# radiocosmology/cora

Hardware: AMD Instinct MI355X
Metric: sky-maps/sec (nside=1024, lmax=2048, 256 freq) (higher is better)
Workload: dtype f64

## Files before the change

cora_amd/csrc/common.h:

```cpp
#pragma once
#include <hip/hip_runtime.h>

#include <cstdarg>
#include <cstdint>
#include <cstdio>
#include <map>
#include <string>
#include <type_traits>
#include <vector>

#include "../../include/corahip.h"

void corahip_set_error(const char *fmt, ...);

struct corahip_prof_entry {
    double total_ms = 0.0;
    int launches = 0;
};

struct corahip_pending_event {
    std::string name;
    hipEvent_t e0, e1;
};

struct corahip_linefft_plan {
    int n = 0, P = 0, logP = 0, blu = 0;
    int Pct = 0;
    double2 *filt_ct = nullptr;
    double2 *tw = nullptr;
    double2 *chirp = nullptr;
    double2 *filt = nullptr;
    double2 *rtw = nullptr;
};

#define CORAHIP_NSCRATCH 12
struct corahip_ctx {
    int device = 0;
    hipStream_t stream = nullptr;
    hipStream_t stream2 = nullptr;
    hipEvent_t ev_fork = nullptr, ev_join = nullptr;
    int *k5_tickets = nullptr;
    unsigned *draw_slot_tab = nullptr;
    int draw_slot_lmax = -1;
    bool mt_plist_ready = false;
    hipStream_t gen_stream = nullptr;
    hipEvent_t ev_ring[8] = {};
    const void *draw_pending = nullptr;
    hipEvent_t t0 = nullptr, t1 = nullptr;
    bool profile = false;
    std::map<std::string, corahip_prof_entry> prof;
    std::vector<corahip_pending_event> pending;
    int num_cu = 256;
    size_t total_mem = 0;
    void *scratch[CORAHIP_NSCRATCH] = {};
    size_t scratch_bytes[CORAHIP_NSCRATCH] = {};
    const void *tt_pin[3] = {nullptr, nullptr, nullptr};
    uint64_t tt_pin_gen = 0;
    bool tt_pinned = false, tt_valid = false;
    hipStream_t tt_stream = nullptr;
    long pairs_key[4] = {-1, -1, -1, -1};
    void *pairs_ptr = nullptr;
    std::map<int, corahip_linefft_plan> linefft;
};

int corahip_ctx_scratch(corahip_ctx *ctx, int slot, size_t bytes, void **out);

struct StageTimer {
    corahip_ctx *ctx;
    hipEvent_t e0 = nullptr, e1 = nullptr;
    const char *name;
    hipStream_t stream;
    StageTimer(corahip_ctx *c, const char *n, hipStream_t on = nullptr, bool other = false) : ctx(c), name(n), stream(other ? on : c->stream) {
        if (ctx->profile) {
            (void)hipEventCreate(&e0);
            (void)hipEventCreate(&e1);
            (void)hipEventRecord(e0, stream);
        }
    }
    ~StageTimer() {
        if (ctx->profile) {
            (void)hipEventRecord(e1, stream);
            ctx->pending.push_back({name, e0, e1});
        }
    }
};

#define HIP_TRY(expr)                                                                       \
    do {                                                                                    \
        hipError_t _e = (expr);                                                             \
        if (_e != hipSuccess) {                                                             \
            corahip_set_error("%s failed: %s (%s:%d)", #expr, hipGetErrorString(_e),        \
                              __FILE__, __LINE__);                                          \
            return (int)_e;                                                                 \
        }                                                                                   \
    } while (0)

#define ARG_CHECK(cond)                                                                     \
    do {                                                                                    \
        if (!(cond)) {                                                                      \
            corahip_set_error("invalid argument: %s (%s:%d)", #cond, __FILE__, __LINE__);   \
            return CORAHIP_EINVAL;                                                          \
        }                                                                                   \
    } while (0)

#define LAUNCH_CHECK() HIP_TRY(hipGetLastError())


static inline unsigned grid_blocks(const corahip_ctx *ctx, long n, int per_cu = 16) {
    long blocks = (n + 255) / 256;
    const long cap = (long)ctx->num_cu * per_cu;
    if (blocks > cap) blocks = cap;
    return (unsigned)(blocks < 1 ? 1 : blocks);
}

static inline void partials_split(long count, int round, int *nb, long *per) {
    long b = (count + 8191) / 8192;
    if (b > 4096) b = 4096;
    long pr = (count + b - 1) / b;
    pr = (pr + round - 1) & ~(long)(round - 1);
    *nb = (int)((count + pr - 1) / pr);
    *per = pr;
}

static inline bool overlaps(const void *a, size_t na, const void *b, size_t nb) {
    const uintptr_t pa = (uintptr_t)a, pb = (uintptr_t)b;
    return a && b && pa < pb + nb && pb < pa + na;
}

static inline int log2_exact(int v) {
    int k = 0;
    while ((1 << k) < v) k++;
    return (1 << k) == v ? k : -1;
}

static inline bool is_aligned(const void *p, unsigned bytes) { return ((uintptr_t)p & (bytes - 1)) == 0; }

__host__ __device__ static inline long nalm_of(int lmax) { return (long)(lmax + 1) * (lmax + 2) / 2; }
__host__ __device__ static inline long alm_idx(int l, int m, int lmax) {
    return (long)m * (2 * lmax + 1 - m) / 2 + l;
}

__device__ static inline long alm_l_of_idx(long idx, int lmax) {
    const double b = 2.0 * lmax + 3.0;
    long m = (long)((b - sqrt(b * b - 8.0 * (double)idx)) * 0.5);
    m = m < 0 ? 0 : (m > lmax ? lmax : m);
    while (m > 0 && m * (2L * lmax + 3 - m) / 2 > idx) m--;
    while (m < lmax && (m + 1) * (2L * lmax + 2 - m) / 2 <= idx) m++;
    return idx - m * (2L * lmax + 1 - m) / 2;
}

typedef double d4_t __attribute__((ext_vector_type(4)));

template <int N, int J = 0, class Fn>
__device__ static inline void static_for(Fn &&f) {
    if constexpr (J < N) {
        f(std::integral_constant<int, J>{});
        static_for<N, J + 1>(f);
    }
}

__device__ static inline void block_sum2(double &a, double &b, double *red) {
#pragma unroll
    for (int o = 32; o >= 1; o >>= 1) {
        a += __shfl_down(a, o, 64);
        b += __shfl_down(b, o, 64);
    }
    const int lane = threadIdx.x & 63, wave = threadIdx.x >> 6;
    if (lane == 0) red[2 * wave] = a, red[2 * wave + 1] = b;
    __syncthreads();
    a = ((red[0] + red[2]) + red[4]) + red[6];
    b = ((red[1] + red[3]) + red[5]) + red[7];
}
```

cora_amd/csrc/ctx.hip:

```cpp
#include "common.h"

#include <cstring>

static thread_local char g_err[512] = "";

void corahip_set_error(const char *fmt, ...) {
    va_list ap;
    va_start(ap, fmt);
    vsnprintf(g_err, sizeof(g_err), fmt, ap);
    va_end(ap);
}

int corahip_ctx_scratch(corahip_ctx *ctx, int slot, size_t bytes, void **out) {
    if (ctx->scratch_bytes[slot] < bytes) {
        HIP_TRY(hipStreamSynchronize(ctx->stream));
        if (ctx->scratch[slot]) HIP_TRY(hipFree(ctx->scratch[slot]));
        ctx->scratch[slot] = nullptr;
        ctx->scratch_bytes[slot] = 0;
        HIP_TRY(hipMalloc(&ctx->scratch[slot], bytes));
        ctx->scratch_bytes[slot] = bytes;
    }
    *out = ctx->scratch[slot];
    return 0;
}

extern "C" {

int corahip_abi_version(void) { return CORAHIP_ABI_VERSION; }

int corahip_abi_minor(void) { return CORAHIP_ABI_MINOR; }

const char *corahip_last_error(void) { return g_err; }

int corahip_device_count(int *count) {
    ARG_CHECK(count != nullptr);
    HIP_TRY(hipGetDeviceCount(count));
    return 0;
}

int corahip_ctx_create(int device_id, corahip_ctx **out) {
    ARG_CHECK(out != nullptr);
    int n = 0;
    HIP_TRY(hipGetDeviceCount(&n));
    ARG_CHECK(device_id >= 0 && device_id < n);
    HIP_TRY(hipSetDevice(device_id));
    hipDeviceProp_t prop;
    HIP_TRY(hipGetDeviceProperties(&prop, device_id));
    if (strncmp(prop.gcnArchName, "gfx950", 6) != 0) {
        corahip_set_error("device %d is %s; libcorahip is built for gfx950 (MI355X) only", device_id,
                          prop.gcnArchName);
        return CORAHIP_ESTATE;
    }
    corahip_ctx *c = new corahip_ctx();
    c->device = device_id;
    c->num_cu = prop.multiProcessorCount;
    c->total_mem = prop.totalGlobalMem;
    HIP_TRY(hipEventCreate(&c->t0));
    HIP_TRY(hipEventCreate(&c->t1));
    *out = c;
    return 0;
}

int corahip_ctx_destroy(corahip_ctx *ctx) {
    if (!ctx) return 0;
    (void)hipStreamSynchronize(ctx->stream);
    for (auto &p : ctx->pending) {
        (void)hipEventDestroy(p.e0);
        (void)hipEventDestroy(p.e1);
    }
    (void)hipEventDestroy(ctx->t0);
    (void)hipEventDestroy(ctx->t1);
    if (ctx->stream2) {
        (void)hipStreamSynchronize(ctx->stream2);
        (void)hipStreamDestroy(ctx->stream2);
        (void)hipEventDestroy(ctx->ev_fork);
        (void)hipEventDestroy(ctx->ev_join);
    }
    if (ctx->gen_stream) {
        (void)hipStreamSynchronize(ctx->gen_stream);
        (void)hipStreamDestroy(ctx->gen_stream);
        for (auto &e : ctx->ev_ring)
            if (e) (void)hipEventDestroy(e);
    }
    for (int i = 0; i < CORAHIP_NSCRATCH; i++)
        if (ctx->scratch[i]) (void)hipFree(ctx->scratch[i]);
    if (ctx->draw_slot_tab) (void)hipFree(ctx->draw_slot_tab);
    if (ctx->k5_tickets) (void)hipFree(ctx->k5_tickets);
    for (auto &kv : ctx->linefft) {
        if (kv.second.tw) (void)hipFree(kv.second.tw);
        if (kv.second.chirp) (void)hipFree(kv.second.chirp);
        if (kv.second.filt) (void)hipFree(kv.second.filt);
        if (kv.second.filt_ct) (void)hipFree(kv.second.filt_ct);
        if (kv.second.rtw) (void)hipFree(kv.second.rtw);
    }
    delete ctx;
    return 0;
}

int corahip_ctx_set_stream(corahip_ctx *ctx, void *hip_stream) {
    ARG_CHECK(ctx != nullptr);
    ctx->stream = (hipStream_t)hip_stream;
    return 0;
}

int corahip_ctx_sync(corahip_ctx *ctx) {
    ARG_CHECK(ctx != nullptr);
    HIP_TRY(hipStreamSynchronize(ctx->stream));
    return 0;
}

int corahip_timer_begin(corahip_ctx *ctx) {
    ARG_CHECK(ctx != nullptr);
    HIP_TRY(hipEventRecord(ctx->t0, ctx->stream));
    return 0;
}

int corahip_timer_end(corahip_ctx *ctx, float *elapsed_ms) {
    ARG_CHECK(ctx != nullptr && elapsed_ms != nullptr);
    HIP_TRY(hipEventRecord(ctx->t1, ctx->stream));
    HIP_TRY(hipEventSynchronize(ctx->t1));
    HIP_TRY(hipEventElapsedTime(elapsed_ms, ctx->t0, ctx->t1));
    return 0;
}

int corahip_profile_enable(corahip_ctx *ctx, int enable) {
    ARG_CHECK(ctx != nullptr);
    ctx->profile = enable != 0;
    return 0;
}

static int drain_pending(corahip_ctx *ctx) {
    if (ctx->pending.empty()) return 0;
    HIP_TRY(hipStreamSynchronize(ctx->stream));
    for (auto &p : ctx->pending) {
        float ms = 0.f;
        HIP_TRY(hipEventElapsedTime(&ms, p.e0, p.e1));
        auto &e = ctx->prof[p.name];
        e.total_ms += ms;
        e.launches += 1;
        (void)hipEventDestroy(p.e0);
        (void)hipEventDestroy(p.e1);
    }
    ctx->pending.clear();
    return 0;
}

int corahip_profile_get(corahip_ctx *ctx, const char *name, double *total_ms, int *launches) {
    ARG_CHECK(ctx != nullptr && name != nullptr);
    int rc = drain_pending(ctx);
    if (rc) return rc;
    auto it = ctx->prof.find(name);
    if (total_ms) *total_ms = it == ctx->prof.end() ? 0.0 : it->second.total_ms;
    if (launches) *launches = it == ctx->prof.end() ? 0 : it->second.launches;
    return 0;
}

int corahip_profile_reset(corahip_ctx *ctx) {
    ARG_CHECK(ctx != nullptr);
    int rc = drain_pending(ctx);
    if (rc) return rc;
    ctx->prof.clear();
    return 0;
}

int corahip_malloc(corahip_ctx *ctx, size_t bytes, void **dptr) {
    ARG_CHECK(ctx != nullptr && dptr != nullptr);
    HIP_TRY(hipSetDevice(ctx->device));
    HIP_TRY(hipMalloc(dptr, bytes));
    return 0;
}

int corahip_free(corahip_ctx *ctx, void *dptr) {
    ARG_CHECK(ctx != nullptr);
    HIP_TRY(hipFree(dptr));
    return 0;
}

int corahip_memcpy_h2d(corahip_ctx *ctx, void *dst, const void *host_src, size_t bytes) {
    ARG_CHECK(ctx != nullptr);
    HIP_TRY(hipMemcpyAsync(dst, host_src, bytes, hipMemcpyHostToDevice, ctx->stream));
    HIP_TRY(hipStreamSynchronize(ctx->stream));
    return 0;
}

int corahip_memcpy_d2h(corahip_ctx *ctx, void *host_dst, const void *src, size_t bytes) {
    ARG_CHECK(ctx != nullptr);
    HIP_TRY(hipMemcpyAsync(host_dst, src, bytes, hipMemcpyDeviceToHost, ctx->stream));
    HIP_TRY(hipStreamSynchronize(ctx->stream));
    return 0;
}

}
```

cora_amd/csrc/draw.hip:

```cpp
#include "common.h"

#include <cstdlib>
#include <type_traits>

#include "rng_dev.h"
#include "stream_internal.h"

__device__ static inline double2 philox_normal_pair(uint64_t seed, int l, int F, int nup, int m,
                                                    const double2 *lg = RNG_LOG_TAB, const double2 *sc = RNG_SC_TAB) {
    const uint64_t ctr = ((uint64_t)((uint32_t)l * (uint32_t)F + (uint32_t)nup) << 32) | (uint32_t)m;
    return philox_boxmuller(ctr, seed, lg, sc);
}

__global__ void normals_kernel(uint64_t seed, int lmax, int F, double *__restrict__ g) {
    const int l = blockIdx.y;
    const int lp1 = l + 1;
    const long n = (long)F * lp1;
    double *gl = g + (size_t)F * l * lp1;
    for (long q = (long)blockIdx.x * blockDim.x + threadIdx.x; q < n; q += (long)gridDim.x * blockDim.x) {
        const int m = (int)(q % lp1);
        const int nup = (int)(q / lp1);
        const double2 v = philox_normal_pair(seed, l, F, nup, m);
        gl[q] = v.x;
        gl[n + q] = v.y;
    }
}

#ifndef DRAW_KK_UNROLL
#define DRAW_KK_UNROLL 2
#endif
#define DRAW_KC 32
#define DRAW_ROWS 64

template <int NCT>
__global__ void __launch_bounds__(256)
draw_kernel(const double *__restrict__ T, size_t t_ldl, int t_row0, const int32_t *__restrict__ info,
            const double *__restrict__ g, size_t g_off, int l_lo, int lmax, int F, int nu0, int nnu, int Gout,
            double *__restrict__ alm) {
    constexpr int NC = 16 * NCT;
    constexpr int STRIDE = DRAW_KC + 2;
    extern __shared__ __attribute__((aligned(16))) double lds[];

    const int l = l_lo + blockIdx.x;
    const int nrow = 2 * (l + 1);
    const int row0 = blockIdx.y * DRAW_ROWS;
    if (row0 >= nrow) return;
    const int col0 = blockIdx.z * NC;
    const int tid = threadIdx.x, lane = tid & 63, wave = tid >> 6;
    const int ri = lane & 15, kq = lane >> 4;
    const int lp1 = l + 1;

    const double *gl = g + ((size_t)F * l * (l + 1) - g_off);
    const double *Tl = T + (size_t)l * t_ldl - (size_t)t_row0 * F;
    const bool dense = (info == nullptr) || (info[l] != 0);

    const int rr = row0 + wave * 16 + ri;
    const bool row_ok = rr < nrow;
    const int c_of = rr >= lp1 ? 1 : 0;
    const int m_of = rr - c_of * lp1;
    const double *grow = gl + (size_t)c_of * F * lp1 + m_of;

    d4_t acc[NCT];
#pragma unroll
    for (int t = 0; t < NCT; t++) acc[t] = (d4_t){0.0, 0.0, 0.0, 0.0};

    const int kmax = dense ? F : min(F, nu0 + col0 + NC);
    for (int k0 = 0; k0 < kmax; k0 += DRAW_KC) {
        __syncthreads();
        for (int it = tid; it < NC * (DRAW_KC / 2); it += 256) {
            const int n = it / (DRAW_KC / 2), q = it % (DRAW_KC / 2);
            const int nu = nu0 + col0 + n;
            double2 v = make_double2(0.0, 0.0);
            const int k = k0 + 2 * q;
            if (col0 + n < nnu && nu < F) {
                if (k + 1 < F) v = *reinterpret_cast<const double2 *>(Tl + (size_t)nu * F + k);
                else if (k < F) v.x = Tl[(size_t)nu * F + k];
            }
            *reinterpret_cast<double2 *>(lds + n * STRIDE + 2 * q) = v;
        }
        __syncthreads();
#pragma unroll
        for (int kk = 0; kk < DRAW_KC / 4; kk++) {
            const int kbase = k0 + 4 * kk;
            if (kbase >= kmax) break;
            const int kp = kbase + kq;
            double a = 0.0;
            if (row_ok && kp < F) a = grow[(size_t)kp * lp1];
            const double *bs = lds + ri * STRIDE + 4 * kk + kq;
#pragma unroll
            for (int t = 0; t < NCT; t++) {
                if (!dense && kbase > nu0 + col0 + 16 * t + 15) continue;
                acc[t] = __builtin_amdgcn_mfma_f64_16x16x4f64(a, bs[16 * t * STRIDE], acc[t], 0, 0, 0);
            }
        }
    }

    const double sc = 0.70710678118654752440;
    const long base = alm_idx(l, 0, lmax);
#pragma unroll
    for (int t = 0; t < NCT; t++) {
        const int col = col0 + 16 * t + ri;
        if (col >= 4 * Gout) continue;
#pragma unroll
        for (int r = 0; r < 4; r++) {
            const int ro = row0 + wave * 16 + kq + 4 * r;
            if (ro < nrow) {
                const int c = ro >= lp1 ? 1 : 0;
                const int m = ro - c * lp1;
                const long idx = (long)m * (2 * lmax + 1 - m) / 2 + l;
                (void)base;
                alm[((size_t)idx * Gout + (col >> 2)) * 8 + c * 4 + (col & 3)] = acc[t][r] * sc;
            }
        }
    }
}

__device__ static inline void draw_glds16(const void *gsrc, unsigned lds_byte_addr) {
    unsigned keep;
    const unsigned dst = __builtin_amdgcn_readfirstlane(lds_byte_addr);
    asm volatile("s_mov_b32 %0, m0\n\ts_mov_b32 m0, %2\n\ts_nop 0\n\tglobal_load_lds_dwordx4 %1, off\n\ts_mov_b32 m0, %0"
                 : "=&s"(keep)
                 : "v"(gsrc), "s"(dst)
                 : "memory");
}

#ifndef DRAW_STAMPS
#define DRAW_STAMPS 0
#endif
#if DRAW_STAMPS
__device__ unsigned long long g_draw_stamps[8];
#define DSTAMP(k) { unsigned long long _t; asm volatile("s_memtime %0\n\ts_waitcnt lgkmcnt(0)" : "=s"(_t)::"memory"); d_acc[k] += _t - d_last; d_last = _t; }
#else
#define DSTAMP(k)
#endif

#define DRAW_WAVES 8
#define DRAW_MB (16 * DRAW_WAVES)
#define DRAW_NBUF 3

static inline long draw_slots(int l_lo, int l_hi) {
    long n = 0;
    for (int l = l_lo; l <= l_hi; l++) n += (l / DRAW_MB) + 1;
    return n;
}

template <int NCT, bool FROMG = false, int NB = DRAW_NBUF>
__global__ void __launch_bounds__(64 * DRAW_WAVES, 2)
draw_rng_kernel(const double *__restrict__ T, size_t t_ldl, int rows, const int32_t *__restrict__ info,
                const double *__restrict__ zeros, uint64_t seed, const double *__restrict__ gsrc, size_t g_off, int l_lo,
                int l_hi, int lmax, int F, int nu0, int nu1, int cw, int nnu, int Gout, int nslots, int ncg0, int ncg,
                double *__restrict__ alm, unsigned *__restrict__ queue, const unsigned *__restrict__ slot_tab) {
    constexpr int NC = 16 * NCT;
    constexpr int ROWD = DRAW_KC;
    constexpr int BUF = NC * ROWD;
    constexpr int QPW = (NC / 4 + DRAW_WAVES - 1) / DRAW_WAVES;
    static_assert(QPW * DRAW_WAVES == NC / 4 || NC / 4 < DRAW_WAVES, "every staging wave issues the same number of pieces");
    extern __shared__ __attribute__((aligned(16))) double lds[];
    static_assert(NB == 3, "the counted waits below assume three stages");
    __shared__ double2 lg_s[257], sc_s[256];
    __shared__ int s_next[2];

    const int tid = threadIdx.x, lane = tid & 63;
    const int wave = __builtin_amdgcn_readfirstlane(tid >> 6);
    const int ri = lane & 15, kq = lane >> 4;
    const int nitems = nslots * ncg;
    const unsigned lds_base = (unsigned)(size_t)(__attribute__((address_space(3))) double *)lds;
#if DRAW_STAMPS
    unsigned long long d_acc[8] = {0, 0, 0, 0, 0, 0, 0, 0}, d_last;
    { unsigned long long _t; asm volatile("s_memtime %0\n\ts_waitcnt lgkmcnt(0)" : "=s"(_t)::"memory"); d_last = _t; }
#endif

    struct item_t {
        int l, mb, base0, lbase, lend, kmax, nchunk, c_full;
        bool tri_tail;
        const double *Tl;
    };
    auto decode = [&](int it) {
        item_t w;
        const int cg = ncg - 1 - it / nslots;
        const int s = it - (it / nslots) * nslots;
        const unsigned e = slot_tab[s];
        const int l = (int)(e >> 8), mb = (int)(e & 255u);
        w.l = l;
        w.mb = mb;
        const bool second = cg >= ncg0;
        w.lbase = second ? cw + (cg - ncg0) * NC : cg * NC;
        w.lend = second ? nnu : min(cw, nnu);
        w.base0 = second ? nu1 + (cg - ncg0) * NC : nu0 + cg * NC;
        const bool dense = (info == nullptr) || (info[l] != 0);
        w.kmax = dense ? F : min(F, w.base0 + NC);
        w.nchunk = (w.kmax + DRAW_KC - 1) / DRAW_KC;
        w.tri_tail = !dense && (w.base0 % DRAW_KC) == 0;
        w.c_full = w.tri_tail ? min(w.nchunk, w.base0 / DRAW_KC) : w.nchunk;
        w.Tl = T + (size_t)l * t_ldl + (size_t)(rows ? w.lbase : w.base0) * F;
        return w;
    };
    auto stage = [&](const item_t &w, int c, int slot) {
        const int k0 = c * DRAW_KC;
#pragma unroll
        for (int it = 0; it < QPW; it++) {
            const int rq = wave + DRAW_WAVES * it;
            if (rq >= NC / 4) break;
            const int n = 4 * rq + (lane >> 4);
            const int slot_dst = lane & 15;
            const int slot_src = slot_dst ^ (n & 15);
            const int nu = w.base0 + n;
            const int k = k0 + 2 * slot_src;
            const double *src = zeros;
            if (w.lbase + n < w.lend && nu < F && k + 1 < F) src = w.Tl + (size_t)n * F + k;
            draw_glds16(src, lds_base + (unsigned)((slot * BUF + 4 * rq * ROWD) * sizeof(double)));
        }
    };

    if constexpr (!FROMG) {
        for (int i = tid; i < 257; i += 64 * DRAW_WAVES) lg_s[i] = RNG_LOG_TAB[i];
        for (int i = tid; i < 256; i += 64 * DRAW_WAVES) sc_s[i] = RNG_SC_TAB[i];
    }

    double a_x[8], a_y[8];
    auto issue_a = [&](const item_t &w, int c, int half, double (&dst)[8]) {
        const int lp1 = w.l + 1;
        const int m = min(w.mb * DRAW_MB + 16 * wave + ri, w.l);
        const double *gre = gsrc + ((size_t)F * w.l * lp1 - g_off) + m;
        const size_t im_off = (size_t)F * lp1;
#pragma unroll
        for (int kk = 0; kk < 4; kk++) {
            const int kp = min(c * DRAW_KC + 16 * half + 4 * kk + kq, F - 1);
            const double *pr = gre + (size_t)kp * lp1;
            const double *pi = pr + im_off;
            asm volatile("global_load_dwordx2 %0, %1, off" : "=v"(dst[2 * kk]) : "v"(pr) : "memory");
            asm volatile("global_load_dwordx2 %0, %1, off" : "=v"(dst[2 * kk + 1]) : "v"(pi) : "memory");
        }
    };
    auto pin_a = [&](double (&dst)[8]) {
#pragma unroll
        for (int i = 0; i < 8; i++) asm volatile("" : "+v"(dst[i]));
    };

    int item = blockIdx.x;
    if (item >= nitems) return;
    item_t w = decode(item);
    int ring = 0, par = 0;
    stage(w, 0, 0);
    if (w.nchunk > 1) stage(w, 1, 1);
    if constexpr (FROMG) {
        if (w.mb * DRAW_MB + 16 * wave < w.l + 1) issue_a(w, 0, 0, a_x);
    }
    DSTAMP(0);

    for (;;) {
        if (tid == 0) s_next[par] = (int)(gridDim.x + atomicAdd(queue, 1u));
        const int l = w.l, lp1 = w.l + 1;
        const int mw = w.mb * DRAW_MB + 16 * wave;
        const bool wave_has_rows = mw < lp1;
        const int m_lane = mw + ri;
        const int kmax = w.kmax, nchunk = w.nchunk;
        d4_t acc0[NCT], acc1[NCT];
#pragma unroll
        for (int t = 0; t < NCT; t++) {
            acc0[t] = (d4_t){0.0, 0.0, 0.0, 0.0};
            acc1[t] = (d4_t){0.0, 0.0, 0.0, 0.0};
        }
        auto half_steps = [&](auto tmin_c, const double *sb, int k0, auto half_c) {
            constexpr int TMIN = decltype(tmin_c)::value;
            constexpr int half = decltype(half_c)::value;
            constexpr int UNR = FROMG ? 4 : DRAW_KK_UNROLL;
#pragma unroll UNR
            for (int kk = 4 * half; kk < 4 * half + 4; kk++) {
                const int kp = k0 + 4 * kk + kq;
                const int kl = 4 * kk + kq;
                double bv[NCT];
                const double *brow = sb + ri * ROWD + 2 * ((kl >> 1) ^ ri) + (kl & 1);
#pragma unroll
                for (int t = TMIN; t < NCT; t++) bv[t] = brow[16 * t * ROWD];
                double2 a;
                if constexpr (FROMG) a = half ? make_double2(a_y[2 * (kk - 4 * half)], a_y[2 * (kk - 4 * half) + 1])
                                              : make_double2(a_x[2 * (kk - 4 * half)], a_x[2 * (kk - 4 * half) + 1]);
                else a = philox_normal_pair(seed, l, F, kp, m_lane, lg_s, sc_s);
#pragma unroll
                for (int t = TMIN; t < NCT; t++) {
                    acc0[t] = __builtin_amdgcn_mfma_f64_16x16x4f64(a.x, bv[t], acc0[t], 0, 0, 0);
                    acc1[t] = __builtin_amdgcn_mfma_f64_16x16x4f64(a.y, bv[t], acc1[t], 0, 0, 0);
                }
            }
        };
        auto mid_chunk = [&](int c) {
            if constexpr (FROMG) {
                constexpr bool ALL_STAGE = QPW * DRAW_WAVES == NC / 4;
                if (c + 2 < nchunk && (ALL_STAGE || wave < NC / 4)) asm volatile("s_waitcnt vmcnt(%0)" ::"n"(QPW) : "memory");
                else asm volatile("s_waitcnt vmcnt(0)" ::: "memory");
                pin_a(a_y);
                if (c + 1 < nchunk) issue_a(w, c + 1, 0, a_x);
            }
        };
        auto chunk_begin = [&](int c) {
            if (FROMG || c == 0 || c + 1 >= nchunk) asm volatile("s_waitcnt vmcnt(0)" ::: "memory");
            else asm volatile("s_waitcnt vmcnt(%0)" ::"n"(QPW) : "memory");
            if constexpr (FROMG) {
                if (wave_has_rows) pin_a(a_x);
            }
            __syncthreads();
#if DRAW_STAMPS
            if (c == 0) { DSTAMP(6); } else
#endif
            DSTAMP(1);
            if constexpr (FROMG) {
                if (wave_has_rows && c * DRAW_KC + 16 < kmax) issue_a(w, c, 1, a_y);
            }
            if (c + NB - 1 < nchunk) stage(w, c + NB - 1, (ring + c + NB - 1) % NB);
            DSTAMP(2);
        };
        int c = 0;
        for (; c < w.c_full; c++) {
            chunk_begin(c);
            if (!wave_has_rows) continue;
            const double *sb = lds + ((ring + c) % NB) * BUF;
            half_steps(std::integral_constant<int, 0>{}, sb, c * DRAW_KC, std::integral_constant<int, 0>{});
            if (c * DRAW_KC + 16 < kmax) {
                mid_chunk(c);
                half_steps(std::integral_constant<int, 0>{}, sb, c * DRAW_KC, std::integral_constant<int, 1>{});
            }
            DSTAMP(3);
        }
        static_for<(NC + DRAW_KC - 1) / DRAW_KC>([&](auto jc) {
            constexpr int J = decltype(jc)::value;
            if (c >= nchunk) return;
            chunk_begin(c);
            if (wave_has_rows) {
                const double *sb = lds + ((ring + c) % NB) * BUF;
                half_steps(std::integral_constant<int, (2 * J < NCT ? 2 * J : NCT)>{}, sb, c * DRAW_KC, std::integral_constant<int, 0>{});
                if (c * DRAW_KC + 16 < kmax) {
                    mid_chunk(c);
                    if constexpr (2 * J + 1 < NCT)
                        half_steps(std::integral_constant<int, (2 * J + 1 < NCT ? 2 * J + 1 : NCT)>{}, sb, c * DRAW_KC,
                                   std::integral_constant<int, 1>{});
                }
                DSTAMP(3);
            }
            c++;
        });

        ring = (ring + nchunk) % NB;
        const int cur_lbase = w.lbase, cur_lend4 = (w.lend + 3) & ~3;
        item = __builtin_amdgcn_readfirstlane(s_next[par]);
        par ^= 1;
        const bool have_next = item < nitems;
        if (have_next) {
            w = decode(item);
            stage(w, 0, ring);
            if (w.nchunk > 1) stage(w, 1, (ring + 1) % NB);
            if constexpr (FROMG) {
                if (w.mb * DRAW_MB + 16 * wave < w.l + 1) issue_a(w, 0, 0, a_x);
            }
        }
        DSTAMP(4);

        if (wave_has_rows) {
            const double sc = 0.70710678118654752440;
            const int q = ri & 3;
            const bool upper = q >= 2;
            auto quad = [](double v, auto ctrl_c) {
                constexpr int CTRL = decltype(ctrl_c)::value;
                int lo = __double2loint(v), hi = __double2hiint(v);
                lo = __builtin_amdgcn_update_dpp(lo, lo, CTRL, 0xF, 0xF, false);
                hi = __builtin_amdgcn_update_dpp(hi, hi, CTRL, 0xF, 0xF, false);
                return __hiloint2double(hi, lo);
            };
#pragma unroll
            for (int t = 0; t < NCT; t++) {
                const int col = cur_lbase + 16 * t + (ri & ~3);
                const bool col_ok = col < cur_lend4;
#pragma unroll
                for (int r = 0; r < 4; r++) {
                    const double re = acc0[t][r] * sc, im = acc1[t][r] * sc;
                    const double re_a = quad(re, std::integral_constant<int, 0x88>{});
                    const double im_a = quad(im, std::integral_constant<int, 0x88>{});
                    const double re_b = quad(re, std::integral_constant<int, 0xDD>{});
                    const double im_b = quad(im, std::integral_constant<int, 0xDD>{});
                    const int m = mw + kq + 4 * r;
                    if (col_ok && m < lp1) {
                        const long idx = (long)m * (2 * lmax + 1 - m) / 2 + l;
                        *reinterpret_cast<double2 *>(alm + ((size_t)idx * Gout + (col >> 2)) * 8 + 2 * q) =
                            upper ? make_double2(im_a, im_b) : make_double2(re_a, re_b);
                    }
                }
            }
        }
        DSTAMP(5);
        if (!have_next) break;
    }
#if DRAW_STAMPS
    if (lane == 0) {
        for (int k = 0; k < 7; k++) atomicAdd(&g_draw_stamps[k], d_acc[k]);
        atomicAdd(&g_draw_stamps[7], 1ull);
    }
#endif
}

struct draw_chan {
    int nu0, nu1, cw, nnu;
};
static int draw_slot_table(corahip_ctx *ctx, int lmax, const unsigned **tab) {
    if (ctx->draw_slot_tab && ctx->draw_slot_lmax == lmax) {
        *tab = ctx->draw_slot_tab;
        return 0;
    }
    std::vector<unsigned> h;
    h.reserve((size_t)draw_slots(0, lmax));
    for (int l = lmax; l >= 0; l--)
        for (int mb = 0; mb <= l / DRAW_MB; mb++) h.push_back(((unsigned)l << 8) | (unsigned)mb);
    if (ctx->draw_slot_tab) (void)hipFree(ctx->draw_slot_tab);
    ctx->draw_slot_tab = nullptr;
    ctx->draw_slot_lmax = -1;
    unsigned *d = nullptr;
    HIP_TRY(hipMalloc((void **)&d, sizeof(unsigned) * h.size()));
    HIP_TRY(hipMemcpy(d, h.data(), sizeof(unsigned) * h.size(), hipMemcpyHostToDevice));
    ctx->draw_slot_tab = d;
    ctx->draw_slot_lmax = lmax;
    *tab = d;
    return 0;
}

template <int NCT, bool FROMG = false, int NB = DRAW_NBUF>
static int launch_draw_rng(corahip_ctx *ctx, hipStream_t stream, const double *T, size_t t_ldl, int rows, const int32_t *info,
                           uint64_t seed, const double *gsrc, size_t g_off, int l_lo, int l_hi, int lmax, int F,
                           draw_chan ch, int Gout, double *alm) {
    constexpr int NC = 16 * NCT;
    const size_t shm = sizeof(double) * NB * NC * DRAW_KC;
    HIP_TRY(hipFuncSetAttribute((const void *)draw_rng_kernel<NCT, FROMG, NB>, hipFuncAttributeMaxDynamicSharedMemorySize,
                                (int)shm));
    char *zq = nullptr;
    int rc = corahip_ctx_scratch(ctx, 3, 8192, (void **)&zq);
    if (rc) return rc;
    HIP_TRY(hipMemsetAsync(zq, 0, 8192, stream));
    const int n0 = std::min(ch.cw, ch.nnu), n1 = ch.nnu - n0;
    const int ncg0 = (((n0 + 3) & ~3) + NC - 1) / NC, ncg = ncg0 + (((n1 + 3) & ~3) + NC - 1) / NC;
    const long nslots = draw_slots(l_lo, l_hi);
    const long nitems = nslots * ncg;
    ARG_CHECK(nitems < (1L << 30) && lmax < (1 << 24) && lmax / DRAW_MB < 256);
    const unsigned *slot_tab = nullptr;
    if ((rc = draw_slot_table(ctx, lmax, &slot_tab))) return rc;
    slot_tab += l_hi < lmax ? draw_slots(l_hi + 1, lmax) : 0;
    const int per_cu = (shm + 8300 > 80 * 1024) ? 1 : 2;
    dim3 grid((unsigned)std::min<long>(nitems, (long)ctx->num_cu * per_cu));
    draw_rng_kernel<NCT, FROMG, NB><<<grid, 64 * DRAW_WAVES, shm, stream>>>(T, t_ldl, rows, info, (const double *)zq, seed, gsrc,
                                                                        g_off, l_lo, l_hi, lmax, F, ch.nu0, ch.nu1, ch.cw,
                                                                        ch.nnu, Gout, (int)nslots, ncg0, ncg, alm,
                                                                        (unsigned *)(zq + 4096), slot_tab);
    LAUNCH_CHECK();
#if DRAW_STAMPS
    {
        unsigned long long hs[8], z[8] = {0};
        HIP_TRY(hipStreamSynchronize(stream));
        HIP_TRY(hipMemcpyFromSymbol(hs, HIP_SYMBOL(g_draw_stamps), sizeof(hs)));
        const double per = 1.0 / (double)std::max<unsigned long long>(hs[7], 1);
        fprintf(stderr, "K3 NCT=%d waves=%llu: cycles/wave  prologue %.0f wait+barrier %.0f (first chunk of an item %.0f) stage-issue %.0f rng+mfma %.0f next-item %.0f epilogue %.0f\n",
                NCT, hs[7], hs[0] * per, hs[1] * per, hs[6] * per, hs[2] * per, hs[3] * per, hs[4] * per, hs[5] * per);
        HIP_TRY(hipMemcpyToSymbol(HIP_SYMBOL(g_draw_stamps), z, sizeof(z)));
    }
#endif
    return 0;
}

__global__ void dev_to_square_kernel(const double *__restrict__ alm, int lmax, int nnu, int G,
                                     double *__restrict__ sq) {
    const int L = lmax + 1;
    const long n = (long)nnu * L * L;
    for (long q = (long)blockIdx.x * blockDim.x + threadIdx.x; q < n; q += (long)gridDim.x * blockDim.x) {
        const int m = (int)(q % L);
        const int l = (int)((q / L) % L);
        const int nu = (int)(q / ((long)L * L));
        double2 v = make_double2(0.0, 0.0);
        if (m <= l) {
            const long idx = (long)m * (2 * lmax + 1 - m) / 2 + l;
            const double *cell = alm + ((size_t)idx * G + (nu >> 2)) * 8 + (nu & 3);
            v = make_double2(cell[0], cell[4]);
        }
        *reinterpret_cast<double2 *>(sq + 2 * q) = v;
    }
}

__global__ void packed_to_dev_kernel(const double *__restrict__ packed, long nalm, int nnu, int G,
                                     double *__restrict__ alm) {
    const long n = nalm * G * 4;
    for (long q = (long)blockIdx.x * blockDim.x + threadIdx.x; q < n; q += (long)gridDim.x * blockDim.x) {
        const int v = (int)(q & 3);
        const int gg = (int)((q >> 2) % G);
        const long idx = q / (4L * G);
        const int nu = 4 * gg + v;
        double2 val = make_double2(0.0, 0.0);
        if (nu < nnu) val = *reinterpret_cast<const double2 *>(packed + 2 * ((size_t)nu * nalm + idx));
        double *cell = alm + ((size_t)idx * G + gg) * 8 + v;
        cell[0] = val.x;
        cell[4] = val.y;
    }
}

template <int NCT>
static int launch_draw(corahip_ctx *ctx, hipStream_t stream, const double *T, size_t t_ldl, int t_row0, const int32_t *info,
                       const double *g, size_t g_off, int l_lo, int l_hi, int lmax, int F, int nu0, int nnu, int Gout,
                       double *alm) {
    constexpr int NC = 16 * NCT;
    const size_t shm = sizeof(double) * NC * (DRAW_KC + 2);
    HIP_TRY(hipFuncSetAttribute((const void *)draw_kernel<NCT>, hipFuncAttributeMaxDynamicSharedMemorySize, (int)shm));
    dim3 grid(l_hi - l_lo + 1, (2 * (l_hi + 1) + DRAW_ROWS - 1) / DRAW_ROWS, (4 * Gout + NC - 1) / NC);
    draw_kernel<NCT><<<grid, 256, shm, stream>>>(T, t_ldl, t_row0, info, g, g_off, l_lo, lmax, F, nu0, nnu, Gout, alm);
    LAUNCH_CHECK();
    return 0;
}

extern "C" {

int corahip_normals_philox(corahip_ctx *ctx, uint64_t seed, int lmax, int F, double *g) {
    ARG_CHECK(ctx != nullptr && g != nullptr && lmax >= 0 && F >= 1);
    StageTimer t(ctx, "normals");
    dim3 grid(std::max(1, std::min(64, (F * (lmax + 1) + 255) / 256)), lmax + 1);
    normals_kernel<<<grid, 256, 0, ctx->stream>>>(seed, lmax, F, g);
    LAUNCH_CHECK();
    return 0;
}

static inline int chan_ncol(const draw_chan &ch) {
    const int n0 = std::min(ch.cw, ch.nnu), n1 = ch.nnu - n0;
    return (std::max(n0, n1) + 3) & ~3;
}
static inline bool chan_folded(const draw_chan &ch) { return ch.nnu > ch.cw; }

static int draw_stream_range(corahip_ctx *ctx, hipStream_t stream, const double *T, int rows, const int32_t *info,
                             const double *g, size_t g_off, int l_lo, int l_hi, int lmax, int F, draw_chan ch,
                             double *alm_dev) {
    const int Gout = (ch.nnu + 3) / 4;
    const size_t t_ldl = rows ? (size_t)ch.nnu * F : (size_t)F * F;
    if (!(F & 1) && !getenv("CORAHIP_DRAW_GENERIC")) {
        const int ncol = chan_ncol(ch);
        if (ncol <= 16) return launch_draw_rng<1, true>(ctx, stream, T, t_ldl, rows, info, 0, g, g_off, l_lo, l_hi, lmax, F, ch, Gout, alm_dev);
        if (ncol <= 32) return launch_draw_rng<2, true>(ctx, stream, T, t_ldl, rows, info, 0, g, g_off, l_lo, l_hi, lmax, F, ch, Gout, alm_dev);
        if (ncol <= 64) return launch_draw_rng<4, true>(ctx, stream, T, t_ldl, rows, info, 0, g, g_off, l_lo, l_hi, lmax, F, ch, Gout, alm_dev);
        return launch_draw_rng<8, true>(ctx, stream, T, t_ldl, rows, info, 0, g, g_off, l_lo, l_hi, lmax, F, ch, Gout, alm_dev);
    }
    ARG_CHECK(!chan_folded(ch));
    const int ncol = 4 * Gout, nu0 = ch.nu0, nnu = ch.nnu, t_row0 = rows ? nu0 : 0;
    if (ncol <= 16) return launch_draw<1>(ctx, stream, T, t_ldl, t_row0, info, g, g_off, l_lo, l_hi, lmax, F, nu0, nnu, Gout, alm_dev);
    if (ncol <= 32) return launch_draw<2>(ctx, stream, T, t_ldl, t_row0, info, g, g_off, l_lo, l_hi, lmax, F, nu0, nnu, Gout, alm_dev);
    if (ncol <= 64) return launch_draw<4>(ctx, stream, T, t_ldl, t_row0, info, g, g_off, l_lo, l_hi, lmax, F, nu0, nnu, Gout, alm_dev);
    if (ncol <= 128) return launch_draw<8>(ctx, stream, T, t_ldl, t_row0, info, g, g_off, l_lo, l_hi, lmax, F, nu0, nnu, Gout, alm_dev);
    return launch_draw<16>(ctx, stream, T, t_ldl, t_row0, info, g, g_off, l_lo, l_hi, lmax, F, nu0, nnu, Gout, alm_dev);
}

static int draw_host_stream(corahip_ctx *ctx, const double *T, int rows, const int32_t *info, const double *g, int lmax, int F,
                            draw_chan ch, double *alm_dev) {
    StageTimer t(ctx, "draw");
    return draw_stream_range(ctx, ctx->stream, T, rows, info, g, 0, 0, lmax, lmax, F, ch, alm_dev);
}

static int draw_philox(corahip_ctx *ctx, const double *T, int rows, const int32_t *info, uint64_t seed, int lmax, int F,
                       draw_chan ch, double *alm_dev) {
    if (F & 1) {
        double *g = nullptr;
        int rc = corahip_ctx_scratch(ctx, 1, sizeof(double) * 2 * (size_t)F * nalm_of(lmax), (void **)&g);
        if (rc) return rc;
        if ((rc = corahip_normals_philox(ctx, seed, lmax, F, g))) return rc;
        return draw_host_stream(ctx, T, rows, info, g, lmax, F, ch, alm_dev);
    }
    StageTimer t(ctx, "draw");
    const int Gout = (ch.nnu + 3) / 4;
    const size_t t_ldl = rows ? (size_t)ch.nnu * F : (size_t)F * F;
    const int ncol = chan_ncol(ch);
    if (ncol <= 16) return launch_draw_rng<1>(ctx, ctx->stream, T, t_ldl, rows, info, seed, nullptr, 0, 0, lmax, lmax, F, ch, Gout, alm_dev);
    if (ncol <= 32) return launch_draw_rng<2>(ctx, ctx->stream, T, t_ldl, rows, info, seed, nullptr, 0, 0, lmax, lmax, F, ch, Gout, alm_dev);
    if (ncol <= 64) return launch_draw_rng<4>(ctx, ctx->stream, T, t_ldl, rows, info, seed, nullptr, 0, 0, lmax, lmax, F, ch, Gout, alm_dev);
    return launch_draw_rng<8>(ctx, ctx->stream, T, t_ldl, rows, info, seed, nullptr, 0, 0, lmax, lmax, F, ch, Gout, alm_dev);
}

static int chan_of(const corahip_chanset *set, int F, draw_chan &ch) {
    ARG_CHECK(set != nullptr && (set->nchunks == 1 || set->nchunks == 2) && set->chunk_nnu >= 1);
    ARG_CHECK(set->nu0[0] >= 0 && set->nu0[0] + set->chunk_nnu <= F);
    if (set->nchunks == 2) {
        ARG_CHECK(set->chunk_nnu % 4 == 0);
        ARG_CHECK(set->nu0[1] >= set->nu0[0] + set->chunk_nnu && set->nu0[1] + set->chunk_nnu <= F);
        ch = draw_chan{set->nu0[0], set->nu0[1], set->chunk_nnu, 2 * set->chunk_nnu};
    } else {
        ch = draw_chan{set->nu0[0], 0, set->chunk_nnu, set->chunk_nnu};
    }
    return 0;
}

int corahip_draw_alm_philox(corahip_ctx *ctx, const double *T, const int32_t *info, uint64_t seed, int lmax, int F,
                            int nu0, int nnu, double *alm_dev) {
    ARG_CHECK(ctx != nullptr && T != nullptr && alm_dev != nullptr);
    ARG_CHECK(lmax >= 0 && F >= 1 && nu0 >= 0 && nnu >= 1 && nu0 + nnu <= F);
    return draw_philox(ctx, T, 0, info, seed, lmax, F, draw_chan{nu0, 0, nnu, nnu}, alm_dev);
}

int corahip_draw_alm_philox_rows(corahip_ctx *ctx, const double *T_rows, const int32_t *info, uint64_t seed, int lmax,
                                 int F, int nu0, int nnu, double *alm_dev) {
    ARG_CHECK(ctx != nullptr && T_rows != nullptr && alm_dev != nullptr);
    ARG_CHECK(lmax >= 0 && F >= 1 && nu0 >= 0 && nnu >= 1 && nu0 + nnu <= F);
    return draw_philox(ctx, T_rows, 1, info, seed, lmax, F, draw_chan{nu0, 0, nnu, nnu}, alm_dev);
}

int corahip_draw_alm_philox_rows_set(corahip_ctx *ctx, const double *T_rows, const int32_t *info, uint64_t seed, int lmax,
                                     int F, const corahip_chanset *set, double *alm_dev) {
    ARG_CHECK(ctx != nullptr && T_rows != nullptr && alm_dev != nullptr && lmax >= 0 && F >= 1);
    draw_chan ch;
    int rc = chan_of(set, F, ch);
    if (rc) return rc;
    ARG_CHECK(!(chan_folded(ch) && (F & 1)));
    return draw_philox(ctx, T_rows, 1, info, seed, lmax, F, ch, alm_dev);
}

int corahip_draw_alm(corahip_ctx *ctx, const double *T, const int32_t *info, const double *g, int lmax, int F,
                     int nu0, int nnu, double *alm_dev) {
    ARG_CHECK(ctx != nullptr && T != nullptr && g != nullptr && alm_dev != nullptr);
    ARG_CHECK(lmax >= 0 && F >= 1 && nu0 >= 0 && nnu >= 1 && nu0 + nnu <= F);
    return draw_host_stream(ctx, T, 0, info, g, lmax, F, draw_chan{nu0, 0, nnu, nnu}, alm_dev);
}

int corahip_draw_alm_rows(corahip_ctx *ctx, const double *T_rows, const int32_t *info, const double *g, int lmax, int F,
                          int nu0, int nnu, double *alm_dev) {
    ARG_CHECK(ctx != nullptr && T_rows != nullptr && g != nullptr && alm_dev != nullptr);
    ARG_CHECK(lmax >= 0 && F >= 1 && nu0 >= 0 && nnu >= 1 && nu0 + nnu <= F);
    return draw_host_stream(ctx, T_rows, 1, info, g, lmax, F, draw_chan{nu0, 0, nnu, nnu}, alm_dev);
}

int corahip_alm_dev_to_square(corahip_ctx *ctx, const double *alm_dev, int lmax, int nnu, double *square) {
    ARG_CHECK(ctx != nullptr && alm_dev != nullptr && square != nullptr && lmax >= 0 && nnu >= 1);
    const long n = (long)nnu * (lmax + 1) * (lmax + 1);
    const int blocks = (int)std::min<long>((n + 255) / 256, 256L * 16);
    dev_to_square_kernel<<<blocks, 256, 0, ctx->stream>>>(alm_dev, lmax, nnu, (nnu + 3) / 4, square);
    LAUNCH_CHECK();
    return 0;
}

int corahip_alm_packed_to_dev(corahip_ctx *ctx, const double *packed, int lmax, int nnu, double *alm_dev) {
    ARG_CHECK(ctx != nullptr && alm_dev != nullptr && packed != nullptr && lmax >= 0 && nnu >= 1);
    const long nalm = nalm_of(lmax);
    const int G = (nnu + 3) / 4;
    const long n = nalm * G * 4;
    const int blocks = (int)std::min<long>((n + 255) / 256, 256L * 16);
    packed_to_dev_kernel<<<blocks, 256, 0, ctx->stream>>>(packed, nalm, nnu, G, alm_dev);
    LAUNCH_CHECK();
    return 0;
}

}

int corahip_draw_range(corahip_ctx *ctx, hipStream_t stream, const double *T, int rows, const int32_t *info, const double *gslot,
                       size_t g_off, int l_lo, int l_hi, int lmax, int F, const corahip_chanset *set, double *alm_dev) {
    draw_chan ch;
    int rc = chan_of(set, F, ch);
    if (rc) return rc;
    return draw_stream_range(ctx, stream, T, rows, info, gslot, g_off, l_lo, l_hi, lmax, F, ch, alm_dev);
}
```

Before: 3214.

## Add wide 256-channel draw kernel with halved m-blocks and double buffering

Adds a specialized draw kernel for more than 128 channel columns. It covers 16 column tiles (256 channels) per item with 8 m-rows per wave and two LDS buffers instead of three. Each Philox normal is then reused across all channels in one pass rather than regenerated per 128-channel group. The slot table becomes per-m-block-size. The cost is higher accumulator register pressure and less latency hiding from the shallower buffer ring.

Result: no change. 3240 (median of 6 runs) (+0.8%).

```diff
diff --git a/cora_amd/csrc/common.h b/cora_amd/csrc/common.h
--- a/cora_amd/csrc/common.h
+++ b/cora_amd/csrc/common.h
@@ -40,8 +40,8 @@
     hipStream_t stream2 = nullptr;
     hipEvent_t ev_fork = nullptr, ev_join = nullptr;
     int *k5_tickets = nullptr;
-    unsigned *draw_slot_tab = nullptr;
-    int draw_slot_lmax = -1;
+    unsigned *draw_slot_tab[2] = {nullptr, nullptr};
+    int draw_slot_lmax[2] = {-1, -1};
     bool mt_plist_ready = false;
     hipStream_t gen_stream = nullptr;
     hipEvent_t ev_ring[8] = {};
diff --git a/cora_amd/csrc/ctx.hip b/cora_amd/csrc/ctx.hip
--- a/cora_amd/csrc/ctx.hip
+++ b/cora_amd/csrc/ctx.hip
@@ -84,7 +84,8 @@
     }
     for (int i = 0; i < CORAHIP_NSCRATCH; i++)
         if (ctx->scratch[i]) (void)hipFree(ctx->scratch[i]);
-    if (ctx->draw_slot_tab) (void)hipFree(ctx->draw_slot_tab);
+    for (auto &t : ctx->draw_slot_tab)
+        if (t) (void)hipFree(t);
     if (ctx->k5_tickets) (void)hipFree(ctx->k5_tickets);
     for (auto &kv : ctx->linefft) {
         if (kv.second.tw) (void)hipFree(kv.second.tw);
diff --git a/cora_amd/csrc/draw.hip b/cora_amd/csrc/draw.hip
--- a/cora_amd/csrc/draw.hip
+++ b/cora_amd/csrc/draw.hip
@@ -138,9 +138,9 @@
 #define DRAW_MB (16 * DRAW_WAVES)
 #define DRAW_NBUF 3
 
-static inline long draw_slots(int l_lo, int l_hi) {
+static inline long draw_slots(int l_lo, int l_hi, int mb = DRAW_MB) {
     long n = 0;
-    for (int l = l_lo; l <= l_hi; l++) n += (l / DRAW_MB) + 1;
+    for (int l = l_lo; l <= l_hi; l++) n += (l / mb) + 1;
     return n;
 }
 
@@ -397,56 +397,273 @@
 #endif
 }
 
+#define DRAW_WIDE_NCT 16
+#define DRAW_WIDE_MB (8 * DRAW_WAVES)
+#define DRAW_WIDE_NBUF 2
+
+__global__ void __launch_bounds__(64 * DRAW_WAVES, 2)
+draw_rng_wide_kernel(const double *__restrict__ T, size_t t_ldl, int rows, const int32_t *__restrict__ info,
+                     const double *__restrict__ zeros, uint64_t seed, int lmax, int F, int nu0, int nu1, int cw, int nnu,
+                     int Gout, int nslots, int ncg0, int ncg, double *__restrict__ alm, unsigned *__restrict__ queue,
+                     const unsigned *__restrict__ slot_tab) {
+    constexpr int NCT = DRAW_WIDE_NCT, NC = 16 * NCT, NB = DRAW_WIDE_NBUF;
+    constexpr int ROWD = DRAW_KC;
+    constexpr int BUF = NC * ROWD;
+    constexpr int QPW = NC / 4 / DRAW_WAVES;
+    static_assert(QPW == NCT / 2, "wave w stages the row quads w + 8 it: piece `it` holds rows of the tiles 2 it, 2 it + 1 only");
+    extern __shared__ __attribute__((aligned(16))) double lds[];
+    __shared__ double2 lg_s[257], sc_s[256];
+    __shared__ int s_next[2];
+
+    const int tid = threadIdx.x, lane = tid & 63;
+    const int wave = __builtin_amdgcn_readfirstlane(tid >> 6);
+    const int ri = lane & 15, kq = lane >> 4;
+    const bool im_lane = ri >= 8;
+    const int nitems = nslots * ncg;
+    const unsigned lds_base = (unsigned)(size_t)(__attribute__((address_space(3))) double *)lds;
+#if DRAW_STAMPS
+    unsigned long long d_acc[8] = {0, 0, 0, 0, 0, 0, 0, 0}, d_last;
+    { unsigned long long _t; asm volatile("s_memtime %0\n\ts_waitcnt lgkmcnt(0)" : "=s"(_t)::"memory"); d_last = _t; }
+#endif
+
+    struct item_t {
+        int l, mb, base0, lbase, lend, nrow, kmax, nchunk, c_full;
+        const double *Tl;
+    };
+    auto decode = [&](int it) {
+        item_t w;
+        const int cg = ncg - 1 - it / nslots;
+        const int s = it - (it / nslots) * nslots;
+        const unsigned e = slot_tab[s];
+        const int l = (int)(e >> 8), mb = (int)(e & 255u);
+        w.l = l;
+        w.mb = mb;
+        const bool second = cg >= ncg0;
+        w.lbase = second ? cw + (cg - ncg0) * NC : cg * NC;
+        w.lend = second ? nnu : min(cw, nnu);
+        w.base0 = second ? nu1 + (cg - ncg0) * NC : nu0 + cg * NC;
+        w.nrow = min(w.lend - w.lbase, F - w.base0);
+        const bool dense = (info == nullptr) || (info[l] != 0);
+        w.kmax = dense ? F : min(F, w.base0 + NC);
+        w.nchunk = (w.kmax + DRAW_KC - 1) / DRAW_KC;
+        const bool tri_tail = !dense && (w.base0 % DRAW_KC) == 0;
+        w.c_full = tri_tail ? min(w.nchunk, w.base0 / DRAW_KC) : w.nchunk;
+        w.Tl = T + (size_t)l * t_ldl + (size_t)(rows ? w.lbase : w.base0) * F;
+        return w;
+    };
+    const int n_lane = 4 * wave + (lane >> 4);
+    const int k_lane = 2 * ((lane & 15) ^ (n_lane & 15));
+    const unsigned src_lane = (unsigned)(n_lane * F + k_lane);
+    auto stage = [&](const item_t &w, int c, int slot) {
+        const int it_min = max(c - w.c_full, 0);
+        const bool k_ok = c * DRAW_KC + k_lane + 1 < F;
+#pragma unroll
+        for (int it = 0; it < QPW; it++) {
+            if (it < it_min) continue;
+            const double *src = w.Tl + (src_lane + (unsigned)(32 * it * F + c * DRAW_KC));
+            if (!(k_ok && 32 * it + n_lane < w.nrow)) src = zeros;
+            draw_glds16(src, lds_base + (unsigned)((slot * BUF + 4 * (wave + DRAW_WAVES * it) * ROWD) * sizeof(double)));
+        }
+    };
+
+    for (int i = tid; i < 257; i += 64 * DRAW_WAVES) lg_s[i] = RNG_LOG_TAB[i];
+    for (int i = tid; i < 256; i += 64 * DRAW_WAVES) sc_s[i] = RNG_SC_TAB[i];
+
+    int item = blockIdx.x;
+    if (item >= nitems) return;
+    item_t w = decode(item);
+    int ring = 0, par = 0;
+    stage(w, 0, 0);
+    DSTAMP(0);
+
+    for (;;) {
+        if (tid == 0) s_next[par] = (int)(gridDim.x + atomicAdd(queue, 1u));
+        const int l = w.l, lp1 = w.l + 1;
+        const int mw = w.mb * DRAW_WIDE_MB + 8 * wave;
+        const bool wave_has_rows = mw < lp1;
+        const int m_lane = mw + (ri & 7);
+        const int kmax = w.kmax, nchunk = w.nchunk;
+        d4_t acc[NCT];
+#pragma unroll
+        for (int t = 0; t < NCT; t++) acc[t] = (d4_t){0.0, 0.0, 0.0, 0.0};
+        auto partner = [](double v) {
+            int lo = __double2loint(v), hi = __double2hiint(v);
+            lo = __builtin_amdgcn_update_dpp(lo, lo, 0x128, 0xF, 0xF, false);
+            hi = __builtin_amdgcn_update_dpp(hi, hi, 0x128, 0xF, 0xF, false);
+            return __hiloint2double(hi, lo);
+        };
+        auto k_step = [&](auto tmin_c, const double *sb, int kl, double a) {
+            constexpr int TMIN = decltype(tmin_c)::value;
+            const double *brow = sb + ri * ROWD + 2 * ((kl >> 1) ^ ri) + (kl & 1);
+            static_for<NCT / 8>([&](auto g_c) {
+                constexpr int T0 = 8 * decltype(g_c)::value > TMIN ? 8 * decltype(g_c)::value : TMIN;
+                constexpr int T1 = 8 * decltype(g_c)::value + 8;
+                if constexpr (T0 < T1) {
+                    double bv[T1 - T0];
+#pragma unroll
+                    for (int t = T0; t < T1; t++) bv[t - T0] = brow[16 * t * ROWD];
+#pragma unroll
+                    for (int t = T0; t < T1; t++) acc[t] = __builtin_amdgcn_mfma_f64_16x16x4f64(a, bv[t - T0], acc[t], 0, 0, 0);
+                }
+            });
+        };
+        auto half_steps = [&](auto tmin_c, const double *sb, int k0, auto half_c) {
+            constexpr int half = decltype(half_c)::value;
+#pragma unroll
+            for (int kk = 4 * half; kk < 4 * half + 4; kk += 2) {
+                const double2 g = philox_normal_pair(seed, l, F, k0 + 4 * (kk + (im_lane ? 1 : 0)) + kq, m_lane, lg_s, sc_s);
+                const double got = partner(im_lane ? g.x : g.y);
+                k_step(tmin_c, sb, 4 * kk + kq, im_lane ? got : g.x);
+                k_step(tmin_c, sb, 4 * kk + 4 + kq, im_lane ? g.y : got);
+            }
+        };
+        auto chunk_begin = [&](int c) {
+            asm volatile("s_waitcnt vmcnt(0)" ::: "memory");
+            __syncthreads();
+#if DRAW_STAMPS
+            if (c == 0) { DSTAMP(6); } else
+#endif
+            DSTAMP(1);
+            if (c + 1 < nchunk) stage(w, c + 1, (ring + c + 1) % NB);
+            DSTAMP(2);
+        };
+        int c = 0;
+        for (; c < w.c_full; c++) {
+            chunk_begin(c);
+            if (!wave_has_rows) continue;
+            const double *sb = lds + ((ring + c) % NB) * BUF;
+            half_steps(std::integral_constant<int, 0>{}, sb, c * DRAW_KC, std::integral_constant<int, 0>{});
+            if (c * DRAW_KC + 16 < kmax) half_steps(std::integral_constant<int, 0>{}, sb, c * DRAW_KC, std::integral_constant<int, 1>{});
+            DSTAMP(3);
+        }
+        static_for<NC / DRAW_KC>([&](auto jc) {
+            constexpr int J = decltype(jc)::value;
+            if (c >= nchunk) return;
+            chunk_begin(c);
+            if (wave_has_rows) {
+                const double *sb = lds + ((ring + c) % NB) * BUF;
+                half_steps(std::integral_constant<int, 2 * J>{}, sb, c * DRAW_KC, std::integral_constant<int, 0>{});
+                if (c * DRAW_KC + 16 < kmax)
+                    half_steps(std::integral_constant<int, 2 * J + 1>{}, sb, c * DRAW_KC, std::integral_constant<int, 1>{});
+                DSTAMP(3);
+            }
+            c++;
+        });
+
+        ring = (ring + nchunk) % NB;
+        const int cur_lbase = w.lbase, cur_lend4 = (w.lend + 3) & ~3;
+        item = __builtin_amdgcn_readfirstlane(s_next[par]);
+        par ^= 1;
+        const bool have_next = item < nitems;
+        if (have_next) {
+            w = decode(item);
+            stage(w, 0, ring);
+        }
+        DSTAMP(4);
+
+        if (wave_has_rows) {
+            const double sc = 0.70710678118654752440;
+            const int q = ri & 3;
+            const bool upper = q >= 2;
+            auto quad = [](double v, auto ctrl_c) {
+                constexpr int CTRL = decltype(ctrl_c)::value;
+                int lo = __double2loint(v), hi = __double2hiint(v);
+                lo = __builtin_amdgcn_update_dpp(lo, lo, CTRL, 0xF, 0xF, false);
+                hi = __builtin_amdgcn_update_dpp(hi, hi, CTRL, 0xF, 0xF, false);
+                return __hiloint2double(hi, lo);
+            };
+#pragma unroll
+            for (int t = 0; t < NCT; t++) {
+                const int col = cur_lbase + 16 * t + (ri & ~3);
+                const bool col_ok = col < cur_lend4;
+#pragma unroll
+                for (int r = 0; r < 2; r++) {
+                    const double re = acc[t][r] * sc, im = acc[t][r + 2] * sc;
+                    const double re_a = quad(re, std::integral_constant<int, 0x88>{});
+                    const double im_a = quad(im, std::integral_constant<int, 0x88>{});
+                    const double re_b = quad(re, std::integral_constant<int, 0xDD>{});
+                    const double im_b = quad(im, std::integral_constant<int, 0xDD>{});
+                    const int m = mw + kq + 4 * r;
+                    if (col_ok && m < lp1) {
+                        const long idx = (long)m * (2 * lmax + 1 - m) / 2 + l;
+                        *reinterpret_cast<double2 *>(alm + ((size_t)idx * Gout + (col >> 2)) * 8 + 2 * q) =
+                            upper ? make_double2(im_a, im_b) : make_double2(re_a, re_b);
+                    }
+                }
+            }
+        }
+        DSTAMP(5);
+        if (!have_next) break;
+    }
+#if DRAW_STAMPS
+    if (lane == 0) {
+        for (int k = 0; k < 7; k++) atomicAdd(&g_draw_stamps[k], d_acc[k]);
+        atomicAdd(&g_draw_stamps[7], 1ull);
+    }
+#endif
+}
+
 struct draw_chan {
     int nu0, nu1, cw, nnu;
 };
-static int draw_slot_table(corahip_ctx *ctx, int lmax, const unsigned **tab) {
-    if (ctx->draw_slot_tab && ctx->draw_slot_lmax == lmax) {
-        *tab = ctx->draw_slot_tab;
+static int draw_slot_table(corahip_ctx *ctx, int lmax, int mbs, const unsigned **tab) {
+    unsigned *&slot_tab = ctx->draw_slot_tab[mbs == DRAW_MB ? 0 : 1];
+    int &slot_lmax = ctx->draw_slot_lmax[mbs == DRAW_MB ? 0 : 1];
+    if (slot_tab && slot_lmax == lmax) {
+        *tab = slot_tab;
         return 0;
     }
     std::vector<unsigned> h;
-    h.reserve((size_t)draw_slots(0, lmax));
+    h.reserve((size_t)draw_slots(0, lmax, mbs));
     for (int l = lmax; l >= 0; l--)
-        for (int mb = 0; mb <= l / DRAW_MB; mb++) h.push_back(((unsigned)l << 8) | (unsigned)mb);
-    if (ctx->draw_slot_tab) (void)hipFree(ctx->draw_slot_tab);
-    ctx->draw_slot_tab = nullptr;
-    ctx->draw_slot_lmax = -1;
+        for (int mb = 0; mb <= l / mbs; mb++) h.push_back(((unsigned)l << 8) | (unsigned)mb);
+    if (slot_tab) (void)hipFree(slot_tab);
+    slot_tab = nullptr;
+    slot_lmax = -1;
     unsigned *d = nullptr;
     HIP_TRY(hipMalloc((void **)&d, sizeof(unsigned) * h.size()));
     HIP_TRY(hipMemcpy(d, h.data(), sizeof(unsigned) * h.size(), hipMemcpyHostToDevice));
-    ctx->draw_slot_tab = d;
-    ctx->draw_slot_lmax = lmax;
+    slot_tab = d;
+    slot_lmax = lmax;
     *tab = d;
     return 0;
 }
 
-template <int NCT, bool FROMG = false, int NB = DRAW_NBUF>
+template <int NCT, bool FROMG = false>
 static int launch_draw_rng(corahip_ctx *ctx, hipStream_t stream, const double *T, size_t t_ldl, int rows, const int32_t *info,
                            uint64_t seed, const double *gsrc, size_t g_off, int l_lo, int l_hi, int lmax, int F,
                            draw_chan ch, int Gout, double *alm) {
-    constexpr int NC = 16 * NCT;
+    constexpr bool WIDE = NCT == DRAW_WIDE_NCT;
+    static_assert(!(WIDE && FROMG), "the 256-channel shape generates its normals");
+    constexpr int NC = 16 * NCT, NB = WIDE ? DRAW_WIDE_NBUF : DRAW_NBUF, MBS = WIDE ? DRAW_WIDE_MB : DRAW_MB;
     const size_t shm = sizeof(double) * NB * NC * DRAW_KC;
-    HIP_TRY(hipFuncSetAttribute((const void *)draw_rng_kernel<NCT, FROMG, NB>, hipFuncAttributeMaxDynamicSharedMemorySize,
-                                (int)shm));
+    const void *kern;
+    if constexpr (WIDE) kern = (const void *)draw_rng_wide_kernel;
+    else kern = (const void *)draw_rng_kernel<NCT, FROMG>;
+    HIP_TRY(hipFuncSetAttribute(kern, hipFuncAttributeMaxDynamicSharedMemorySize, (int)shm));
     char *zq = nullptr;
     int rc = corahip_ctx_scratch(ctx, 3, 8192, (void **)&zq);
     if (rc) return rc;
     HIP_TRY(hipMemsetAsync(zq, 0, 8192, stream));
     const int n0 = std::min(ch.cw, ch.nnu), n1 = ch.nnu - n0;
     const int ncg0 = (((n0 + 3) & ~3) + NC - 1) / NC, ncg = ncg0 + (((n1 + 3) & ~3) + NC - 1) / NC;
-    const long nslots = draw_slots(l_lo, l_hi);
+    const long nslots = draw_slots(l_lo, l_hi, MBS);
     const long nitems = nslots * ncg;
-    ARG_CHECK(nitems < (1L << 30) && lmax < (1 << 24) && lmax / DRAW_MB < 256);
+    ARG_CHECK(nitems < (1L << 30) && lmax < (1 << 24) && lmax / MBS < 256);
     const unsigned *slot_tab = nullptr;
-    if ((rc = draw_slot_table(ctx, lmax, &slot_tab))) return rc;
-    slot_tab += l_hi < lmax ? draw_slots(l_hi + 1, lmax) : 0;
+    if ((rc = draw_slot_table(ctx, lmax, MBS, &slot_tab))) return rc;
+    slot_tab += l_hi < lmax ? draw_slots(l_hi + 1, lmax, MBS) : 0;
     const int per_cu = (shm + 8300 > 80 * 1024) ? 1 : 2;
     dim3 grid((unsigned)std::min<long>(nitems, (long)ctx->num_cu * per_cu));
-    draw_rng_kernel<NCT, FROMG, NB><<<grid, 64 * DRAW_WAVES, shm, stream>>>(T, t_ldl, rows, info, (const double *)zq, seed, gsrc,
-                                                                        g_off, l_lo, l_hi, lmax, F, ch.nu0, ch.nu1, ch.cw,
-                                                                        ch.nnu, Gout, (int)nslots, ncg0, ncg, alm,
-                                                                        (unsigned *)(zq + 4096), slot_tab);
+    if constexpr (WIDE)
+        draw_rng_wide_kernel<<<grid, 64 * DRAW_WAVES, shm, stream>>>(T, t_ldl, rows, info, (const double *)zq, seed, lmax, F, ch.nu0,
+                                                                     ch.nu1, ch.cw, ch.nnu, Gout, (int)nslots, ncg0, ncg, alm,
+                                                                     (unsigned *)(zq + 4096), slot_tab);
+    else
+        draw_rng_kernel<NCT, FROMG><<<grid, 64 * DRAW_WAVES, shm, stream>>>(T, t_ldl, rows, info, (const double *)zq, seed, gsrc,
+                                                                            g_off, l_lo, l_hi, lmax, F, ch.nu0, ch.nu1, ch.cw,
+                                                                            ch.nnu, Gout, (int)nslots, ncg0, ncg, alm,
+                                                                            (unsigned *)(zq + 4096), slot_tab);
     LAUNCH_CHECK();
 #if DRAW_STAMPS
     {
@@ -569,7 +786,8 @@
     if (ncol <= 16) return launch_draw_rng<1>(ctx, ctx->stream, T, t_ldl, rows, info, seed, nullptr, 0, 0, lmax, lmax, F, ch, Gout, alm_dev);
     if (ncol <= 32) return launch_draw_rng<2>(ctx, ctx->stream, T, t_ldl, rows, info, seed, nullptr, 0, 0, lmax, lmax, F, ch, Gout, alm_dev);
     if (ncol <= 64) return launch_draw_rng<4>(ctx, ctx->stream, T, t_ldl, rows, info, seed, nullptr, 0, 0, lmax, lmax, F, ch, Gout, alm_dev);
-    return launch_draw_rng<8>(ctx, ctx->stream, T, t_ldl, rows, info, seed, nullptr, 0, 0, lmax, lmax, F, ch, Gout, alm_dev);
+    if (ncol <= 128) return launch_draw_rng<8>(ctx, ctx->stream, T, t_ldl, rows, info, seed, nullptr, 0, 0, lmax, lmax, F, ch, Gout, alm_dev);
+    return launch_draw_rng<DRAW_WIDE_NCT>(ctx, ctx->stream, T, t_ldl, rows, info, seed, nullptr, 0, 0, lmax, lmax, F, ch, Gout, alm_dev);
 }
 
 static int chan_of(const corahip_chanset *set, int F, draw_chan &ch) {
```
